# foriequal0/homework-18-graphics-raytracer

Hardware: AMD Instinct MI355X
Metric: Mrays/s (primary+secondary) at 1920x1080, depth 8 (higher is better)
Workload: dtype f32

## Files before the change

### homework-18-graphics-raytracer_amd/csrc/rt_pwf.hip

```cpp
#include "rt_pwf_kernel.h"

namespace rt {

static size_t pwf_dynamic_lds(uint32_t node_cap, uint32_t ring_cap) {
    const bool packed = pa_ready_packed(node_cap, ring_cap);
    return (size_t)(PA_READY_WORDS((node_cap + 63u) / 64u, packed) + 2u * PA_READY_WORDS(ring_cap / 64u, packed)) * sizeof(uint32_t);
}

int pwf_workgroups_per_cu(uint32_t node_cap, uint32_t ring_cap, bool bfs_walk) {
    int n = 0;
    const size_t lds = pwf_dynamic_lds(node_cap, ring_cap);
    const bool packed = pa_ready_packed(node_cap, ring_cap);
    const hipError_t e = bfs_walk ? (packed ? hipOccupancyMaxActiveBlocksPerMultiprocessor(&n, pwf_kernel<true, true>, (int)PA_THREADS, lds)
                                            : hipOccupancyMaxActiveBlocksPerMultiprocessor(&n, pwf_kernel<false, true>, (int)PA_THREADS, lds))
                                  : (packed ? hipOccupancyMaxActiveBlocksPerMultiprocessor(&n, pwf_kernel<true, false>, (int)PA_THREADS, lds)
                                            : hipOccupancyMaxActiveBlocksPerMultiprocessor(&n, pwf_kernel<false, false>, (int)PA_THREADS, lds));
    if (e != hipSuccess || n < 1) n = 1;
    return n;
}

__global__ void pwf_init_kernel(uint32_t *global, KernelFrame *frame, const KernelFrame fr) {
    if (threadIdx.x < PW_G_BLOCK_WORDS) global[threadIdx.x] = 0u;
    if (threadIdx.x == 0u) *frame = fr;
}

size_t pwf_arena_bytes(uint32_t node_cap, uint32_t ring_cap, uint32_t max_depth) {
    return ((size_t)node_cap * 4u + (size_t)ring_cap * (3u + PA_SHADE_U4)) * sizeof(uint4) + (size_t)(node_cap / 64u) * 2u * sizeof(uint32_t) +
           (((size_t)node_cap + 15u) & ~(size_t)15u) + (size_t)pwf_fold_list_regions(max_depth) * node_cap * sizeof(uint32_t) + 256u;
}

#ifdef PA_STATS
static uint32_t *g_pw_last_global = nullptr;
extern "C" int rt_diag_read_pwf(uint32_t *out32) {
    if (!g_pw_last_global) return -1;
    return hipMemcpy(out32, g_pw_last_global, 32 * sizeof(uint32_t), hipMemcpyDeviceToHost) == hipSuccess ? 0 : -1;
}
extern "C" int rt_diag_read_pwf_phases(unsigned long long *out32, int reset) {
    if (hipMemcpyFromSymbol(out32, HIP_SYMBOL(pa_phase_stats), 32 * sizeof(unsigned long long)) != hipSuccess) return -1;
    if (reset) {
        unsigned long long zero[32] = {0};
        if (hipMemcpyToSymbol(HIP_SYMBOL(pa_phase_stats), zero, sizeof zero) != hipSuccess) return -1;
    }
    return 0;
}
#endif

hipError_t launch_pwf(const KernelScene &sc, KernelFrame fr, float *out, const PwParams &pp, uint32_t workgroups, hipStream_t stream,
                      bool init, bool first_band, bool last_band) {
    const uint32_t total = fr.cols * fr.rows;
    fr.n_chunks = (total + 63u) / 64u;
    if (total == 0u) return hipSuccess;
#ifdef PA_STATS
    g_pw_last_global = pp.global;
#endif
    if (init) hipLaunchKernelGGL(pwf_init_kernel, dim3(1), dim3(64), 0, stream, pp.global, const_cast<KernelFrame *>(pp.frame), fr);
    if (first_band) record_main_kernel_event(0, stream);
    const size_t lds = pwf_dynamic_lds(pp.node_cap, pp.ring_cap);
    const bool packed = pa_ready_packed(pp.node_cap, pp.ring_cap);
    if (frame_is_rays(fr)) launch_pwf_rays(sc, pp, out, workgroups, lds, stream, packed, sc.bfs_walk != 0u && pp.bfs_scratch != nullptr);
    else launch_pwf_kernel<false>(sc, pp, out, workgroups, lds, stream, packed, sc.bfs_walk != 0u && pp.bfs_scratch != nullptr);
    if (last_band) record_main_kernel_event(1, stream);
    return hipGetLastError();
}

}

#ifdef RT_DIAG_STAGES
RT_DIAG_STAGE_READER(rt_diag_read_stages_pwf)
#endif
#ifdef RT_DIAG_NEED
RT_DIAG_NEED_READER(rt_diag_read_need_pwf)
#endif
#ifdef RT_DIAG_BFS
RT_DIAG_BFS_READER(rt_diag_read_bfs)
#endif
```

### homework-18-graphics-raytracer_amd/csrc/rt_pwf_common.h

```cpp
#ifndef RT_PWF_COMMON_H
#define RT_PWF_COMMON_H

#include <hip/hip_runtime.h>
#include <stdint.h>

#include "rt_shade.h"
#include "rt_kernels.h"
#include "rt_cast.h"

namespace rt {

#define PW_NO_CHILD 0xffffffffu
#define PW_FINAL 0xfffffffeu
#define PW_DEPTH_SHIFT 21u
#define PW_MODE_SHIFT 27u
#define PW_EXCL_MASK (0xe0000000u | ((1u << PW_DEPTH_SHIFT) - 1u))


__device__ __forceinline__ uint32_t pfu(float x) { return __float_as_uint(x); }
__device__ __forceinline__ float puf(uint32_t x) { return __uint_as_float(x); }

__device__ __forceinline__ uint32_t lds_append(uint32_t *counter, bool want) {
    const unsigned long long mask = __builtin_amdgcn_ballot_w64(want);
    if (mask == 0ull) return 0u;
// ... 67 lines not shown
        const uint32_t c = w & 0xffffu;
        if (c == 64u || (w & PA_SEALED) != 0u) {
            if (atomicCAS(&q->taken, page, page + 1u) == page) {
                ready[page & page_mask] = 0u;
                *start = page * 64u;
                return c;
            }
            continue;
        }
        if (min_partial == 0u || a >= (page + 1u) * 64u || c < min_partial || c != a - page * 64u) return 0u;
        if (atomicCAS(&q->alloc, a, (page + 1u) * 64u) == a) atomicOr(&ready[page & page_mask], PA_SEALED);
    }
    return 0u;
}

PA_HELPER uint32_t pa_try_append(PaQueue *q, const uint32_t *released, uint32_t capacity, bool want, bool *ok) {
    const unsigned long long mask = __builtin_amdgcn_ballot_w64(want);
    *ok = true;
    if (mask == 0ull) return 0u;
    const uint32_t n = (uint32_t)__builtin_popcountll(mask);
    const int leader = (int)__builtin_ctzll(mask);
    uint32_t base = 0xffffffffu;
    if ((int)(threadIdx.x & 63u) == leader) {
        for (int tries = 0; tries < 4; ++tries) {
            const uint32_t a = lds_load(&q->alloc);
            if (a + n - (lds_load(released) << 6) > capacity) break;
            if (atomicCAS(&q->alloc, a, a + n) == a) { base = a; break; }
        }
    }
    base = (uint32_t)__builtin_amdgcn_readlane((int)base, leader);
    if (base == 0xffffffffu) { *ok = false; return 0u; }
    return base + __builtin_amdgcn_mbcnt_hi((uint32_t)(mask >> 32), __builtin_amdgcn_mbcnt_lo((uint32_t)mask, 0u));
}

PA_HELPER uint32_t pa_try_append_some(PaQueue *q, const uint32_t *released, uint32_t capacity, bool want, bool *ok) {
    const unsigned long long mask = __builtin_amdgcn_ballot_w64(want);
    *ok = false;
    if (mask == 0ull) return 0u;
    const uint32_t n = (uint32_t)__builtin_popcountll(mask);
    const int leader = (int)__builtin_ctzll(mask);
    uint32_t base = 0u, take = 0u;
    if ((int)(threadIdx.x & 63u) == leader) {
        for (int tries = 0; tries < 4; ++tries) {
            const uint32_t a = lds_load(&q->alloc);
            const uint32_t used = a - (lds_load(released) << 6);
            const uint32_t t = used >= capacity ? 0u : (capacity - used < n ? capacity - used : n);
            if (t == 0u) break;
            if (atomicCAS(&q->alloc, a, a + t) == a) { base = a; take = t; break; }
        }
    }
    base = (uint32_t)__builtin_amdgcn_readlane((int)base, leader);
    take = (uint32_t)__builtin_amdgcn_readlane((int)take, leader);
    const uint32_t rank = __builtin_amdgcn_mbcnt_hi((uint32_t)(mask >> 32), __builtin_amdgcn_mbcnt_lo((uint32_t)mask, 0u));
    *ok = want && rank < take;
    return base + rank;
}

template <bool PACKED = false>
PA_HELPER void pa_publish(uint32_t *ready, uint32_t page_mask, bool want, uint32_t pos, uint32_t *gen) {
    const unsigned long long mask = __builtin_amdgcn_ballot_w64(want);
    if (mask == 0ull) return;
    __builtin_amdgcn_fence(__ATOMIC_RELEASE, "workgroup");
    const uint32_t n = (uint32_t)__builtin_popcountll(mask);
    const int leader = (int)__builtin_ctzll(mask);
    const uint32_t first = (uint32_t)__builtin_amdgcn_readlane((int)pos, leader);
    if ((int)(threadIdx.x & 63u) == leader) {
        const uint32_t p0 = first >> 6, p1 = (first + n - 1u) >> 6;
        if (PACKED) {
            const uint32_t i0 = p0 & page_mask, i1 = p1 & page_mask;
            const uint32_t n0 = p0 == p1 ? n : (p1 << 6) - first;
            atomicAdd(&ready[i0 >> 1], n0 << pa_ready_shift(i0));
            if (p0 != p1) atomicAdd(&ready[i1 >> 1], (n - n0) << pa_ready_shift(i1));
        } else if (p0 == p1) {
            atomicAdd(&ready[p0 & page_mask], n);
        } else {
            const uint32_t n0 = (p1 << 6) - first;
            atomicAdd(&ready[p0 & page_mask], n0);
            atomicAdd(&ready[p1 & page_mask], n - n0);
        }
        atomicAdd(gen, 1u);
    }
}

template <class Scene>
__device__ __forceinline__ bool next_shadow_ray(const Scene &sc, uint32_t *light_i, V3 pos, V3 adj_n, DirLight *dl) {
    while (*light_i < sc.n_lights) {
        V3 direction;
        if (light_asks(sc.lights[*light_i], sc.light_aux[*light_i], pos, adj_n, &direction)) {
            (void)approximate_into_directional(sc.lights[*light_i], pos, dl);
            return true;
        }
        *light_i += 1u;
    }
    return false;
}

template <class Scene>
__device__ __forceinline__ bool next_shadow_ray_in_step(const Scene &sc, uint32_t first, bool searching, uint32_t *light_i, V3 pos, V3 adj_n) {
    bool found = false;
    for (uint32_t li = first; li < sc.n_lights; ++li) {
        if (__builtin_amdgcn_ballot_w64(searching) == 0ull) break;
        V3 direction;
        const bool asks = light_asks(uniform_ref(sc.lights + li), uniform_ref(sc.light_aux + li), pos, adj_n, &direction);
        if (searching && asks) {
            *light_i = li;
            found = true;
            searching = false;
        }
    }
    return found;
}

}

#endif
```

### homework-18-graphics-raytracer_amd/csrc/rt_pwf_kernel.h

```cpp
#ifndef RT_PWF_KERNEL_H
#define RT_PWF_KERNEL_H

#include <hip/hip_runtime.h>
#include <stdint.h>

#include "../../include/rt_amd.h"
#include "rt_device_scene.h"
#include "rt_shade.h"
#include "rt_kernels.h"
#include "rt_cast.h"
#include "rt_pwf_common.h"

namespace rt {

#ifndef PA_WAVES
#define PA_WAVES 8u
#endif
#define PA_THREADS (PA_WAVES * 64u)
#ifndef PA_MIN_WAVES
#define PA_MIN_WAVES 6
#endif
#ifndef PA_SHADE_PAGES
#define PA_SHADE_PAGES 4u
#endif
#ifndef PA_MIN_PARTIAL
#define PA_MIN_PARTIAL 1u
#endif
#ifndef PA_CHAIN_PARTIAL_MIN
#define PA_CHAIN_PARTIAL_MIN 1u
#endif
#ifndef PA_PRIO_CHAIN
#define PA_PRIO_CHAIN 1
#define PA_PRIO_TILE 1
#endif
#ifndef PA_SLEEP
#define PA_SLEEP 16
#endif
#define PA_SHADE_U4 5u
#ifndef PA_LDS_PAGES
#define PA_LDS_PAGES 2u
#endif
#ifndef PA_LQ
#define PA_LQ 3u
#endif
#define PA_LQ_SHIFT 4u
#ifndef PA_LDS_F_PAGES
#define PA_LDS_F_PAGES 2u
#endif
#ifndef PA_LDS_N_PAGES
#define PA_LDS_N_PAGES 2u
#endif
#ifndef PA_DRAIN_ROOM
#define PA_DRAIN_ROOM 64u
#endif
#define PA_IN_LDS 8u
#define PA_SPIN_LIMIT (1u << 22)

enum : uint32_t { PA_T_NONE = 0u, PA_T_NODE = 1u, PA_T_REFR = 2u, PA_T_TILE = 3u, PA_T_SHADE = 4u };

struct PaShared {
    PaQueue n, f, s;
    PaQueue l[PA_LQ];
    uint32_t l_released[PA_LQ];
    uint32_t ready_l[PA_LQ][PA_LDS_PAGES];
    PaQueue lf;
    uint32_t lf_released;
    uint32_t ready_lf[PA_LDS_F_PAGES];
    PaQueue ln;
    uint32_t ln_released;
    uint32_t ready_ln[PA_LDS_N_PAGES];
    uint32_t root_alloc;
    uint32_t tiles_exhausted;
    uint32_t tile_list_count;
    uint32_t static_next;
    uint32_t idle;
    uint32_t gen;
    uint32_t done;
    uint32_t abort;
    uint32_t fold_count[64];
};

template <class P>
__device__ __forceinline__ void pa_store_shade(P *t, uint32_t id, uint32_t prim, uint32_t word, V3 spos, V3 adj_n, V3 in_dir, V3 sdiffuse, V3 sum) {
    t[PA_F(0u)] = make_uint4(id, prim, word, 0u);
    t[PA_F(1u)] = make_uint4(pfu(spos.x), pfu(spos.y), pfu(spos.z), pfu(sum.x));
    t[PA_F(2u)] = make_uint4(pfu(adj_n.x), pfu(adj_n.y), pfu(adj_n.z), pfu(sum.y));
    t[PA_F(3u)] = make_uint4(pfu(in_dir.x), pfu(in_dir.y), pfu(in_dir.z), pfu(sum.z));
    t[PA_F(4u)] = make_uint4(pfu(sdiffuse.x), pfu(sdiffuse.y), pfu(sdiffuse.z), 0u);
}

template <class P>
__device__ __forceinline__ void pa_store_node(P *t, V3 o, V3 d, uint32_t word, float contribution, uint32_t id) {
    t[PA_F(0u)] = make_uint4(pfu(o.x), pfu(o.y), pfu(o.z), pfu(d.x));
    t[PA_F(1u)] = make_uint4(pfu(d.y), pfu(d.z), word, pfu(contribution));
    if (id != 0xffffffffu) t[PA_F(2u)] = make_uint4(id, 0u, 0u, 0u);
}

__device__ __forceinline__ uint32_t pa_top_node(uint32_t *root_alloc, const uint32_t *n_alloc, uint32_t node_cap, bool want, bool *overflow) {
    const unsigned long long mask = __builtin_amdgcn_ballot_w64(want);
    *overflow = false;
    if (mask == 0ull) return 0u;
    const uint32_t n = (uint32_t)__builtin_popcountll(mask);
    const int leader = (int)__builtin_ctzll(mask);
    uint32_t base = 0u;
    if ((int)(threadIdx.x & 63u) == leader) base = atomicAdd(root_alloc, n);
    base = (uint32_t)__builtin_amdgcn_readlane((int)base, leader);
    if (base + n + lds_load(n_alloc) > node_cap) { *overflow = want; return 0u; }
    return node_cap - 1u - (base + __builtin_amdgcn_mbcnt_hi((uint32_t)(mask >> 32), __builtin_amdgcn_mbcnt_lo((uint32_t)mask, 0u)));
}

template <class P>
__device__ __forceinline__ void pa_store_refr(P *t, V3 o, V3 d, uint32_t word, uint32_t parent, uint32_t obj, float contribution, float travel, uint32_t retry) {
    t[PA_F(0u)] = make_uint4(pfu(o.x), pfu(o.y), pfu(o.z), pfu(d.x));
    t[PA_F(1u)] = make_uint4(pfu(d.y), pfu(d.z), word, parent);
    t[PA_F(2u)] = make_uint4(obj, pfu(contribution), pfu(travel), retry);
}

__device__ __forceinline__ void pa_release_page(uint32_t *released, uint32_t page, uint32_t lane) {
    asm volatile("s_waitcnt lgkmcnt(0)" ::: "memory");
    if (lane == 0u) {
        while (lds_load(released) != page) __builtin_amdgcn_s_sleep(1);
        __hip_atomic_store(released, page + 1u, __ATOMIC_RELEASE, __HIP_MEMORY_SCOPE_WORKGROUP);
    }
}

#ifdef PA_STATS
__device__ unsigned long long pa_phase_stats[32];
#define PA_TICK() __builtin_readcyclecounter()
#endif

template <bool PACKED, bool BFS = false, bool RAYS = false>
__global__ __launch_bounds__(PA_THREADS, BFS ? 2 : PA_MIN_WAVES) void pwf_kernel(const KernelScene sc, const PwParams pp, float *__restrict__ out) {
    BfsLds *bfs_lds = nullptr;
    BfsScratch bfs_ws = {nullptr, nullptr, nullptr, 0u, 0u};
    if constexpr (BFS) {
        __shared__ BfsLds bfs_lds_all[PA_WAVES];
        bfs_lds = &bfs_lds_all[threadIdx.x >> 6];
        uint2 *const mine = reinterpret_cast<uint2 *>(pp.bfs_scratch) + ((size_t)blockIdx.x * PA_WAVES + (threadIdx.x >> 6)) * (2u * (size_t)pp.bfs_items_cap + pp.bfs_jobs_cap);
        bfs_ws.items_a = mine;
        bfs_ws.items_b = mine + pp.bfs_items_cap;
        bfs_ws.jobs = mine + 2u * (size_t)pp.bfs_items_cap;
        bfs_ws.items_cap = pp.bfs_items_cap;
        bfs_ws.jobs_cap = pp.bfs_jobs_cap;
    }
    extern __shared__ uint32_t pa_ready[];
    __shared__ PaShared S;
    __shared__ uint4 lds_shade[PA_LQ * PA_LDS_PAGES * PA_SHADE_U4 * 64u];
    __shared__ uint4 lds_refr[PA_LDS_F_PAGES * 3u * 64u];
    __shared__ uint4 lds_node[PA_LDS_N_PAGES * 3u * 64u];
    const auto &fr = uniform_ref(pp.frame);
    const uint32_t lane = threadIdx.x & 63u;
    const uint32_t total_slots = fr.cols * fr.rows;
    const uint32_t n_tiles = fr.n_chunks;
    const float THRESHOLD = 0.001f;

    unsigned char *arena = pp.arena + (size_t)blockIdx.x * pp.arena_stride;
    uint4 *node_in = reinterpret_cast<uint4 *>(arena);
    uint4 *nodes = node_in + (size_t)pp.node_cap * 2u;
    uint4 *shade_q = nodes + (size_t)pp.node_cap * 2u;
    uint4 *refr_q = shade_q + (size_t)pp.ring_cap * PA_SHADE_U4;
    uint32_t *tile_list = reinterpret_cast<uint32_t *>(refr_q + (size_t)pp.ring_cap * 3u);
    const uint32_t ring_mask = pp.ring_cap - 1u;
    const uint32_t tile_cap = pp.node_cap / 64u;
    unsigned char *root_mark = reinterpret_cast<unsigned char *>(((uintptr_t)(tile_list + (size_t)tile_cap * 2u) + 15u) & ~(uintptr_t)15u);
    uint32_t *fold_list = reinterpret_cast<uint32_t *>(root_mark + (((size_t)pp.node_cap + 15u) & ~(size_t)15u));
    auto fold_slot = [&](uint32_t level, uint32_t i) -> uint32_t * {
        uint32_t *region = fold_list + (size_t)((level - 1u) >> 1) * pp.node_cap;
        return region + (((level - 1u) & 1u) != 0u ? pp.node_cap - 1u - i : i);
    };
    const uint32_t node_pages = (pp.node_cap + 63u) / 64u, ring_pages = pp.ring_cap / 64u;
    uint32_t *ready_n = pa_ready, *ready_s = pa_ready + PA_READY_WORDS(node_pages, PACKED), *ready_f = ready_s + PA_READY_WORDS(ring_pages, PACKED);
    const uint32_t ring_page_mask = ring_pages - 1u;

    for (uint32_t i = threadIdx.x; i < PA_READY_WORDS(node_pages, PACKED) + 2u * PA_READY_WORDS(ring_pages, PACKED); i += PA_THREADS) pa_ready[i] = 0u;
    if (threadIdx.x < 64u) S.fold_count[threadIdx.x] = 0u;
    if (threadIdx.x == 0u) {
        S.n.alloc = S.n.taken = 0u;
        S.f.alloc = S.f.taken = 0u;
        S.s.alloc = S.s.taken = 0u;
        for (uint32_t q = 0; q < PA_LQ; ++q) {
            S.l[q].alloc = S.l[q].taken = 0u;
            S.l_released[q] = 0u;
            for (uint32_t k = 0; k < PA_LDS_PAGES; ++k) S.ready_l[q][k] = 0u;
        }
        S.lf.alloc = S.lf.taken = 0u;
        S.lf_released = 0u;
        for (uint32_t k = 0; k < PA_LDS_F_PAGES; ++k) S.ready_lf[k] = 0u;
        S.ln.alloc = S.ln.taken = 0u;
        S.ln_released = 0u;
        for (uint32_t k = 0; k < PA_LDS_N_PAGES; ++k) S.ready_ln[k] = 0u;
        S.root_alloc = 0u;
        S.tiles_exhausted = 0u;
        S.tile_list_count = 0u;
        S.static_next = 0u;
        S.idle = 0u;
        S.gen = 0u;
        S.done = 0u;
        S.abort = 0u;
    }
    __syncthreads();
    uint32_t casts = 0u;
    auto queue_shade = [&](bool want, uint32_t id, uint32_t prim, uint32_t word, uint32_t light_i, V3 spos, V3 adj_n, V3 in_dir, V3 sdiffuse, V3 sum) {
        const uint32_t mine = light_i < PA_LQ - 1u ? light_i : PA_LQ - 1u;
#pragma unroll
        for (uint32_t q = 0; q < PA_LQ; ++q) {
            const bool w = want && mine == q;
            if (__builtin_amdgcn_ballot_w64(w) == 0ull) continue;
            bool fits;
            const uint32_t k = pa_try_append_some(&S.l[q], &S.l_released[q], PA_LDS_PAGES * 64u, w, &fits);
            if (fits) pa_store_shade(lds_shade + q * (PA_LDS_PAGES * PA_SHADE_U4 * 64u) + pa_entry(k & (PA_LDS_PAGES * 64u - 1u), PA_SHADE_U4), id, prim, word, spos, adj_n, in_dir, sdiffuse, sum);
            pa_publish(S.ready_l[q], PA_LDS_PAGES - 1u, fits, k, &S.gen);
            want = want && !fits;
        }
#ifdef PA_STATS
        for (uint32_t q = 0; q < 3u; ++q) {
            const unsigned long long m = __builtin_amdgcn_ballot_w64(want && (mine < 2u ? mine : 2u) == q);
            if (m != 0ull && lane == (uint32_t)__builtin_ctzll(m)) atomicAdd(pp.global + 28 + q, (uint32_t)__builtin_popcountll(m));
        }
#endif
        const uint32_t k = lds_append(&S.s.alloc, want);
        if (want) pa_store_shade(shade_q + pa_entry(k & ring_mask, PA_SHADE_U4), id, prim, word, spos, adj_n, in_dir, sdiffuse, sum);
        pa_publish<PACKED>(ready_s, ring_page_mask, want, k, &S.gen);
    };
#ifdef PA_STATS
    const unsigned long long st_t0 = __builtin_amdgcn_s_memrealtime();
    uint32_t st_hist[5] = {0u, 0u, 0u, 0u, 0u};
    uint32_t st_shadow[3] = {0u, 0u, 0u};
    unsigned long long ph[26];
    for (int k = 0; k < 26; ++k) ph[k] = 0ull;
#endif

    for (;;) {
        if (lds_load(&S.done) != 0u || lds_load(&S.abort) != 0u) break;

#ifdef PA_STATS
        const unsigned long long ph_t0 = PA_TICK();
#endif
        uint32_t type = PA_T_NONE, start = 0u, count = 0u;
        if (lane == 0u) {
            const uint32_t gen = lds_load(&S.gen);
            auto look = [&]() -> uint32_t {
                const uint32_t a0 = lds_load(&S.ln.alloc), a1 = lds_load(&S.n.alloc), a2 = lds_load(&S.lf.alloc), a3 = lds_load(&S.f.alloc);
                const uint32_t t0 = lds_load(&S.ln.taken), t1 = lds_load(&S.n.taken), t2 = lds_load(&S.lf.taken), t3 = lds_load(&S.f.taken);
                uint32_t al[PA_LQ], tl[PA_LQ];
                for (uint32_t q = 0; q < PA_LQ; ++q) { al[q] = lds_load(&S.l[q].alloc); tl[q] = lds_load(&S.l[q].taken); }
                const uint32_t as = lds_load(&S.s.alloc), ts = lds_load(&S.s.taken);
                uint32_t m = (a0 > t0 * 64u ? 1u : 0u) | (a1 > t1 * 64u ? 2u : 0u) | (a2 > t2 * 64u ? 4u : 0u) | (a3 > t3 * 64u ? 8u : 0u);
                for (uint32_t q = 0; q < PA_LQ; ++q) m |= al[q] > tl[q] * 64u ? 16u << q : 0u;
                m |= as > ts * 64u ? 16u << PA_LQ : 0u;
                return m;
            };
            uint32_t have = look();
            auto claim_chain = [&](uint32_t min_partial) {
                if ((have & 1u) != 0u) {
                    count = pa_claim(&S.ln, S.ready_ln, PA_LDS_N_PAGES - 1u, min_partial, &start);
                    if (count != 0u) { type = PA_T_NODE | PA_IN_LDS; return; }
                }
                if ((have & 2u) != 0u) {
                    count = pa_claim<PACKED>(&S.n, ready_n, 0xffffffffu, min_partial, &start);
                    if (count != 0u) { type = PA_T_NODE; return; }
                }
                if ((have & 4u) != 0u) {
                    count = pa_claim(&S.lf, S.ready_lf, PA_LDS_F_PAGES - 1u, min_partial, &start);
                    if (count != 0u) { type = PA_T_REFR | PA_IN_LDS; return; }
                }
                if ((have & 8u) != 0u) {
                    count = pa_claim<PACKED>(&S.f, ready_f, ring_page_mask, min_partial, &start);
                    if (count != 0u) type = PA_T_REFR;
                }
            };
            auto claim_shade = [&](uint32_t min_partial) {
                for (uint32_t q = 0; q < PA_LQ; ++q) {
                    if ((have & (16u << q)) == 0u) continue;
                    count = pa_claim(&S.l[q], S.ready_l[q], PA_LDS_PAGES - 1u, min_partial, &start);
                    if (count != 0u) { type = PA_T_SHADE | PA_IN_LDS | (q << PA_LQ_SHIFT); return; }
                }
                if ((have & (16u << PA_LQ)) == 0u) return;
                count = pa_claim<PACKED>(&S.s, ready_s, ring_page_mask, min_partial, &start);
                if (count != 0u) type = PA_T_SHADE;
            };
            claim_chain(0u);
            if (PA_DRAIN_ROOM != 0u && type == PA_T_NONE && lds_load(&S.tiles_exhausted) == 0u) {
                for (uint32_t q = 0; q < PA_LQ; ++q) {
                    if (lds_load(&S.l[q].alloc) - (lds_load(&S.l_released[q]) << 6) + PA_DRAIN_ROOM > PA_LDS_PAGES * 64u) {
                        count = pa_claim(&S.l[q], S.ready_l[q], PA_LDS_PAGES - 1u, 0u, &start);
                        if (count != 0u) { type = PA_T_SHADE | PA_IN_LDS | (q << PA_LQ_SHIFT); break; }
                    }
                }
            }
            if (PA_CHAIN_PARTIAL_MIN != 0u && type == PA_T_NONE) claim_chain(PA_CHAIN_PARTIAL_MIN);
            bool tried_tile = false;
            for (int pass = 0; pass < 2 && type == PA_T_NONE; ++pass) {
                if (!tried_tile && lds_load(&S.tiles_exhausted) == 0u) {
                    uint32_t shade_pages = (lds_load(&S.s.alloc) >> 6) - lds_load(&S.s.taken);
                    for (uint32_t q = 0; q < PA_LQ; ++q) shade_pages += (lds_load(&S.l[q].alloc) >> 6) - lds_load(&S.l[q].taken);
                    if (pass == 1 || (int32_t)shade_pages < (int32_t)PA_SHADE_PAGES) {
                        tried_tile = true;
                        const uint32_t used = lds_load(&S.n.alloc) + lds_load(&S.root_alloc);
                        const uint32_t room = pp.node_cap > used ? pp.node_cap - used : 0u;
                        if (room < 64u * pp.tile_reserve || lds_load(&S.tile_list_count) >= tile_cap) {
                            S.tiles_exhausted = 1u;
                        } else {
                            const uint32_t share = n_tiles / gridDim.x;
                            const uint32_t own = share / 2u > (share < 8u ? share : 8u) ? share / 2u : (share < 8u ? share : 8u);
                            uint32_t k;
                            const uint32_t mine = own != 0u && lds_load(&S.static_next) < own ? atomicAdd(&S.static_next, 1u) : own;
                            if (mine < own) k = blockIdx.x + gridDim.x * mine;
                            else k = gridDim.x * own + atomicAdd(pp.global + PW_G_TILE, 1u);
                            if (k >= n_tiles) {
                                S.tiles_exhausted = 1u;
                            } else {
                                start = pp.tile_order != nullptr ? pp.tile_order[k] : (uint32_t)(((unsigned long long)k * pp.tile_stride) % n_tiles);
                                count = total_slots - start * 64u < 64u ? total_slots - start * 64u : 64u;
                                type = PA_T_TILE;
                            }
                        }
                    }
                }
                if (type == PA_T_NONE && pass == 0) claim_shade(0u);
            }
            for (int last = 0; last < 2 && type == PA_T_NONE; ++last) {
                const uint32_t min_partial = last ? 1u : PA_MIN_PARTIAL;
                have = look();
                claim_chain(min_partial);
                if (type != PA_T_NONE) break;
                claim_shade(min_partial);
                if (type != PA_T_NONE) break;
                if (last) {
                    if (lds_load(&S.idle) == PA_WAVES - 1u) S.done = 1u;
                    break;
                }
                if (atomicAdd(&S.idle, 1u) + 1u == PA_WAVES) {
                    atomicSub(&S.idle, 1u);
                    continue;
                }
                uint32_t spins = 0u;
                while (lds_load(&S.gen) == gen && lds_load(&S.done) == 0u && lds_load(&S.abort) == 0u) {
                    __builtin_amdgcn_s_sleep(PA_SLEEP);
                    if (++spins > PA_SPIN_LIMIT) {
                        S.abort = 1u;
                        atomicExch(pp.global + PW_G_OVERFLOW, 1u);
                    }
                }
                atomicSub(&S.idle, 1u);
                break;
            }
        }
        type = (uint32_t)__builtin_amdgcn_readfirstlane((int)type);
        start = (uint32_t)__builtin_amdgcn_readfirstlane((int)start);
        count = (uint32_t)__builtin_amdgcn_readfirstlane((int)count);
        const bool in_lds = (type & PA_IN_LDS) != 0u;
        const uint32_t lq = (type >> PA_LQ_SHIFT) & 3u;
        type &= 7u;
        const bool one_light = type == PA_T_SHADE && in_lds && (lq < PA_LQ - 1u || sc.n_lights <= PA_LQ);
#ifdef PA_STATS
        const unsigned long long ph_t1 = PA_TICK();
        if (type == PA_T_NONE) ph[24] += ph_t1 - ph_t0;
        const uint32_t ph_k = type == PA_T_NODE ? 0u : (type == PA_T_REFR ? 1u : (type == PA_T_TILE ? 2u : 3u));
#endif
        if (type == PA_T_NONE) continue;
        __builtin_amdgcn_fence(__ATOMIC_ACQUIRE, "workgroup");
        if (type == PA_T_SHADE) __builtin_amdgcn_s_setprio(0);
        else if (type == PA_T_TILE) __builtin_amdgcn_s_setprio(PA_PRIO_TILE);
        else __builtin_amdgcn_s_setprio(PA_PRIO_CHAIN);
#ifdef PA_STATS
        st_hist[count <= 8u ? 0 : (count <= 16u ? 1 : (count <= 32u ? 2 : (count < 64u ? 3 : 4)))] += 1u;
#endif

        const bool active = lane < count;
        Ray req;
        req.o = v3(0.0f, 0.0f, 0.0f);
        req.d = v3(0.0f, 0.0f, 1.0f);
        req.mode = FACE_FRONT;
        req.excl = 0u;
        bool do_cast = active;
        uint32_t id = 0u;
        uint32_t depth = 0u;
        float contribution = 1.0f;
        uint32_t obj = 0u;
        float travel = 0.0f;
        int32_t retry = -1;
        uint32_t prim = 0u, light_i = 0u, sflags = 0u;
        V3 spos = v3(0.0f, 0.0f, 0.0f), adj_n = v3(0.0f, 0.0f, 1.0f), in_dir = v3(0.0f, 0.0f, 1.0f), sdiffuse = spos, sum = spos;
        DirLight dl;
        dl.direction = dl.color = v3(0.0f, 0.0f, 0.0f);
        bool from_tile = false;

        if (type == PA_T_TILE) {
            const uint32_t tile = start;
            uint32_t base = 0u, entry = 0u;
            if (lane == 0u) {
                base = atomicAdd(&S.root_alloc, count);
                entry = atomicAdd(&S.tile_list_count, 1u);
            }
            base = (uint32_t)__builtin_amdgcn_readfirstlane((int)base);
            entry = (uint32_t)__builtin_amdgcn_readfirstlane((int)entry);
            if (base + count + lds_load(&S.n.alloc) > pp.node_cap || entry >= tile_cap) {
                if (lane == 0u) { S.abort = 1u; atomicExch(pp.global + PW_G_OVERFLOW, 1u); }
                break;
            }
            const uint32_t first_id = pp.node_cap - base - count;
            if (lane == 0u) { tile_list[entry * 2u] = tile; tile_list[entry * 2u + 1u] = first_id; }
            id = first_id + lane;
            depth = (uint32_t)(fr.max_depth > 0 ? fr.max_depth : 0);
            if constexpr (RAYS) {
                contribution = frame_root_contribution(fr);
                if (active) req = ray_from_abi(frame_rays(fr) + (tile * 64u + lane), sc.n_triangles, sc.n_spheres);
                do_cast = active && !(contribution < THRESHOLD);
            } else if (active) {
                uint32_t row, col;
                pw_slot_to_pixel(fr, tile * 64u + lane, &row, &col);
                const uint32_t x = fr.x0 + col, y = fr.y0 + row * fr.y_step;
                const float clip_y = (fr.half_height - (float)y) / fr.height_f;
                const float clip_x = ((float)x - fr.half_width) / fr.height_f;
                const V3 cx = v3(fr.cam_x[0], fr.cam_x[1], fr.cam_x[2]);
                const V3 cy = v3(fr.cam_y[0], fr.cam_y[1], fr.cam_y[2]);
                const V3 ct = v3(fr.cam_toward[0], fr.cam_toward[1], fr.cam_toward[2]);
                req.o = v3(fr.cam_origin[0], fr.cam_origin[1], fr.cam_origin[2]);
                req.d = normalize(clip_x * cx + clip_y * cy + ct);
            }
            type = PA_T_NODE;
            from_tile = true;
        } else if (type == PA_T_NODE) {
            uint4 a, b;
            a = b = make_uint4(0u, 0u, 0u, 0u);
            if (in_lds) {
                if (active) {
                    const uint4 *t = lds_node + pa_entry((start + lane) & (PA_LDS_N_PAGES * 64u - 1u), 3u);
                    a = t[PA_F(0u)], b = t[PA_F(1u)];
                    id = t[PA_F(2u)].x;
                }
                pa_release_page(&S.ln_released, start >> 6, lane);
            } else {
                id = start + lane;
                if (active) a = node_in[pa_entry(id, 2u)], b = node_in[pa_entry(id, 2u) + PA_F(1u)];
            }
            if (active) {
                req.o = v3(puf(a.x), puf(a.y), puf(a.z));
                req.d = v3(puf(a.w), puf(b.x), puf(b.y));
                req.mode = (b.z >> PW_MODE_SHIFT) & 3u;
                depth = (b.z >> PW_DEPTH_SHIFT) & 63u;
                req.excl = b.z & PW_EXCL_MASK;
                contribution = puf(b.w);
            }
        } else if (type == PA_T_REFR) {
            uint4 a, b, c;
            a = b = c = make_uint4(0u, 0u, 0u, 0u);
            if (in_lds) {
                if (active) {
                    const uint4 *t = lds_refr + pa_entry((start + lane) & (PA_LDS_F_PAGES * 64u - 1u), 3u);
                    a = t[PA_F(0u)], b = t[PA_F(1u)], c = t[PA_F(2u)];
                }
                pa_release_page(&S.lf_released, start >> 6, lane);
            } else if (active) {
                const uint4 *t = refr_q + pa_entry((start + lane) & ring_mask, 3u);
                a = t[PA_F(0u)], b = t[PA_F(1u)], c = t[PA_F(2u)];
            }
            if (active) {
                req.o = v3(puf(a.x), puf(a.y), puf(a.z));
                req.d = v3(puf(a.w), puf(b.x), puf(b.y));
                req.mode = (b.z >> PW_MODE_SHIFT) & 3u;
                depth = (b.z >> PW_DEPTH_SHIFT) & 63u;
                req.excl = b.z & PW_EXCL_MASK;
                id = b.w;
                obj = c.x;
                contribution = puf(c.y);
                travel = puf(c.z);
                retry = (int32_t)c.w;
            }
        } else {
            uint4 a, b, c, d, e;
            a = b = c = d = e = make_uint4(0u, 0u, 0u, 0u);
            if (in_lds) {
                if (active) {
                    const uint4 *t = lds_shade + lq * (PA_LDS_PAGES * PA_SHADE_U4 * 64u) + pa_entry((start + lane) & (PA_LDS_PAGES * 64u - 1u), PA_SHADE_U4);
                    a = t[PA_F(0u)], b = t[PA_F(1u)], c = t[PA_F(2u)], d = t[PA_F(3u)], e = t[PA_F(4u)];
                }
                pa_release_page(&S.l_released[lq], start >> 6, lane);
            } else if (active) {
                const uint4 *t = shade_q + pa_entry((start + lane) & ring_mask, PA_SHADE_U4);
                a = t[PA_F(0u)], b = t[PA_F(1u)], c = t[PA_F(2u)], d = t[PA_F(3u)], e = t[PA_F(4u)];
            }
            if (active) {
                id = a.x; prim = a.y; obj = a.z & 0xffffu; light_i = (a.z >> 16) & 0x3fffu; sflags = a.z >> 30;
                spos = v3(puf(b.x), puf(b.y), puf(b.z)); sum.x = puf(b.w);
                adj_n = v3(puf(c.x), puf(c.y), puf(c.z)); sum.y = puf(c.w);
                in_dir = v3(puf(d.x), puf(d.y), puf(d.z)); sum.z = puf(d.w);
                sdiffuse = v3(puf(e.x), puf(e.y), puf(e.z));
                if (one_light) do_cast = approximate_into_directional(uniform_ref(sc.lights + lq), spos, &dl);
                else do_cast = next_shadow_ray(sc, &light_i, spos, adj_n, &dl);
                req.o = spos;
                req.d = -dl.direction;
                req.mode = FACE_BACK;
                req.excl = pack_excl(prim, FACE_BACK);
            }
        }

#ifdef PA_STATS
        const unsigned long long ph_t2 = PA_TICK();
#endif
        CastResult cr;
        cr.prim = -1;
        cr.t = 0.0f;
        cr.bf = 0u;
        cr.a0 = cr.a1 = cr.a2 = 0.0f;
        if constexpr (BFS) {
            cr = cast_bfs(sc, req, do_cast, bfs_lds, bfs_ws);
            if (do_cast) casts += 1u;
        } else if (do_cast) {
            cr = cast_asm(sc, req);
            casts += 1u;
        }
#ifdef PA_STATS
        const unsigned long long ph_t3 = PA_TICK();
#endif

        if (type == PA_T_NODE) {
            V3 acc = v3(0.0f, 0.0f, 0.0f);
            float rc = 0.0f, fc = 0.0f;
            uint32_t rec_cr = PW_FINAL, rec_cf = PW_NO_CHILD;
            bool want_shade = false, want_refl = false, want_refr = false;
            HitGeom nh;
            nh.pos = nh.normal = v3(0.0f, 0.0f, 0.0f);
            nh.u = nh.v = 0.0f;
            nh.prim = nh.bf = nh.obj = 0u;
            V3 inside_d = v3(0.0f, 0.0f, 0.0f);
            if (active && cr.prim >= 0) {
                nh = finish_hit(sc, req, cr, false);
                const rt_material &rm = sc.materials[nh.obj];
                const float shade_contribution = (1.0f - rm.shiness) * (1.0f - rm.transparency);
                want_shade = contribution * shade_contribution >= THRESHOLD;
                if (depth > 0u) {
                    acc = v3(0.0f, 0.0f, 0.0f) * shade_contribution;
                    rc = rm.shiness * (1.0f - rm.transparency);
                    fc = rm.transparency;
                    rec_cr = PW_NO_CHILD;
                    want_refl = contribution * rc >= THRESHOLD;
                    if (contribution * fc > THRESHOLD) {
                        V3 refract_in;
                        if (refract_dir(nh.normal, req.d, rm.refraction_index, &refract_in)) {
                            inside_d = normalize(refract_in);
                            want_refr = true;
                        }
                    }
                }
            }
            bool refl_in_lds, overflow;
            const uint32_t q_refl = pa_try_append(&S.ln, &S.ln_released, PA_LDS_N_PAGES * 64u, want_refl, &refl_in_lds);
            const uint32_t k_refl = refl_in_lds ? pa_top_node(&S.root_alloc, &S.n.alloc, pp.node_cap, want_refl, &overflow)
                                                : lds_append(&S.n.alloc, want_refl);
            if (!refl_in_lds) overflow = want_refl && k_refl + lds_load(&S.root_alloc) >= pp.node_cap;
            if (want_refl && !overflow) rec_cr = k_refl;
            const bool below = active && cr.prim >= 0 && depth > 0u && (want_refl || want_refr);
            const bool bare = active && cr.prim >= 0 && depth > 0u && !below;
            if (active) {
                if (below) nodes[pa_entry(id, 2u) + PA_F(1u)] = make_uint4(pfu(fc), 0u, rec_cr, rec_cf);
                if (from_tile) root_mark[id] = (unsigned char)(below ? 0u : 0xffu);
            }
            if (want_refl && !overflow) {
                const V3 d = reflect_dir(nh.normal, req.d);
                const uint32_t word = pack_excl(nh.prim, nh.bf ? FACE_FRONT : FACE_BACK) | (req.mode << PW_MODE_SHIFT) | ((depth - 1u) << PW_DEPTH_SHIFT);
                if (refl_in_lds) pa_store_node(lds_node + pa_entry(q_refl & (PA_LDS_N_PAGES * 64u - 1u), 3u), nh.pos, d, word, contribution * rc, k_refl);
                else pa_store_node(node_in + pa_entry(k_refl, 2u), nh.pos, d, word, contribution * rc, 0xffffffffu);
            }
// ... 244 lines not shown
                    const uint32_t nv = total_slots - first_slot < 64u ? total_slots - first_slot : 64u;
                    live[j] = lane < nv;
                    id[j] = base + lane;
                    slot[j] = first_slot + lane;
                }
                if (live[j]) {
                    ra[j] = nodes[pa_entry(id[j], 2u)];
                    rb[j] = make_uint4(0u, 0u, PW_FINAL, PW_NO_CHILD);
                    if (root_mark[id[j]] != 0xffu) rb[j] = nodes[pa_entry(id[j], 2u) + PA_F(1u)];
                }
            }
            if (pp.tile_cost != nullptr) {
#pragma unroll
                for (uint32_t j = 0; j < 4u; ++j) {
                    const unsigned long long deep = __builtin_amdgcn_ballot_w64(live[j] && rb[j].z != PW_FINAL);
                    if (lane == 0u && tile_of[j] != 0xffffffffu) pp.tile_cost[tile_of[j]] = (uint32_t)__builtin_popcountll(deep);
                }
            }
            uint4 cr4[4], cf4[4];
#pragma unroll
            for (uint32_t j = 0; j < 4u; ++j) {
                cr4[j] = cf4[j] = make_uint4(0u, 0u, 0u, 0u);
                if (live[j] && rb[j].z != PW_FINAL) {
                    if (rb[j].z != PW_NO_CHILD) cr4[j] = nodes[pa_entry(rb[j].z, 2u)];
                    if (rb[j].w != PW_NO_CHILD) cf4[j] = nodes[pa_entry(rb[j].w, 2u)];
                }
            }
#pragma unroll
            for (uint32_t j = 0; j < 4u; ++j) {
                if (!live[j]) continue;
                const uint4 a = ra[j], b = rb[j];
                V3 value = v3(puf(a.x), puf(a.y), puf(a.z));
                if (b.z != PW_FINAL) {
                    const float rc = puf(a.w), fc = puf(b.x), decay = puf(b.y);
                    V3 reflection = v3(0.0f, 0.0f, 0.0f), refraction = v3(0.0f, 0.0f, 0.0f);
                    if (b.z != PW_NO_CHILD) reflection = v3(puf(cr4[j].x), puf(cr4[j].y), puf(cr4[j].z));
                    if (b.w != PW_NO_CHILD) refraction = v3(puf(cf4[j].x), puf(cf4[j].y), puf(cf4[j].z)) * decay;
                    value = (value + reflection * rc) + refraction * fc;
                }
                uint32_t row, col;
                pw_slot_to_pixel(fr, slot[j], &row, &col);
                float *px = out + ((size_t)row * fr.cols + col) * 3u;
                if constexpr (RAYS) {
                    px[0] = value.x;
                    px[1] = value.y;
                    px[2] = value.z;
                } else {
                    px[0] = 0.0f + value.x;
                    px[1] = 0.0f + value.y;
                    px[2] = 0.0f + value.z;
                }
            }
        }
        if (threadIdx.x == 0u && n_started != 0u) atomicAdd(pp.global + PW_G_TILES_DONE, n_started);
#ifdef PA_STATS
        __syncthreads();
        if (threadIdx.x == 0u) {
            atomicAdd(&pa_phase_stats[26], st_f0 - st_t2);
            atomicAdd(&pa_phase_stats[27], st_f1 - st_f0);
            atomicAdd(&pa_phase_stats[28], __builtin_amdgcn_s_memrealtime() - st_f1);
            atomicAdd(&pa_phase_stats[29], 1ull);
        }
#endif
    }
#ifdef PA_STATS
    __syncthreads();
    {
        const unsigned long long st_t3 = __builtin_amdgcn_s_memrealtime();
        if (lane == 0u) { atomicAdd(pp.global + 8, (uint32_t)(st_t1 - st_t0)); atomicMax(pp.global + 9, (uint32_t)(st_t1 - st_t0)); }
        if (lane == 0u) for (int k = 0; k < 5; ++k) atomicAdd(pp.global + 20 + k, st_hist[k]);
        for (int k = 0; k < 3; ++k) {
            uint32_t v = st_shadow[k];
            for (int off = 32; off > 0; off >>= 1) v += __shfl_down(v, off, 64);
            if (lane == 0u && v != 0u) atomicAdd(pp.global + (k == 0 ? 18 : (k == 1 ? 19 : 31)), v);
        }
        if (lane == 0u) {
            ph[25] = st_t3 - st_t2;
            for (int k = 0; k < 26; ++k) atomicAdd(&pa_phase_stats[k], ph[k]);
        }
        if (threadIdx.x == 0u) {
            atomicAdd(pp.global + 10, (uint32_t)(st_t2 - st_t0)); atomicMax(pp.global + 11, (uint32_t)(st_t2 - st_t0));
            atomicAdd(pp.global + 12, (uint32_t)(st_t3 - st_t2)); atomicMax(pp.global + 13, (uint32_t)(st_t3 - st_t2));
            atomicAdd(pp.global + 14, 1u); atomicAdd(pp.global + 15, S.n.alloc);
            atomicAdd(pp.global + 25, S.s.alloc); atomicAdd(pp.global + 26, S.f.alloc); atomicAdd(pp.global + 27, S.root_alloc);
            atomicMin(pp.global + 16, (uint32_t)(st_t3 - st_t0)); atomicMax(pp.global + 17, (uint32_t)(st_t3 - st_t0));
        }
    }
#endif
    if (threadIdx.x == 0u) S.gen = 0u;
    __syncthreads();
    for (int off = 32; off > 0; off >>= 1) casts += __shfl_down(casts, off, 64);
    if (lane == 0u && casts != 0u) atomicAdd(&S.gen, casts);

    __syncthreads();
    if (threadIdx.x == 0u) {
        if (S.gen != 0u) atomicAdd(reinterpret_cast<unsigned long long *>(pp.global + PW_G_CASTS), (unsigned long long)S.gen);
        __threadfence();
        if (atomicAdd(pp.global + PW_G_GROUPS_DONE, 1u) + 1u == gridDim.x) {
            __threadfence();
            uint32_t overflow = __hip_atomic_load(pp.global + PW_G_OVERFLOW, __ATOMIC_RELAXED, __HIP_MEMORY_SCOPE_AGENT);
            const uint32_t tiles_done = __hip_atomic_load(pp.global + PW_G_TILES_DONE, __ATOMIC_RELAXED, __HIP_MEMORY_SCOPE_AGENT);
            if (overflow == 0u && tiles_done != n_tiles) {
                overflow = 1u;
                atomicExch(pp.global + PW_G_OVERFLOW, 1u);
            }
            if (overflow == 0u && pp.ray_count != nullptr)
                atomicAdd(pp.ray_count,
                          __hip_atomic_load(reinterpret_cast<unsigned long long *>(pp.global + PW_G_CASTS), __ATOMIC_RELAXED, __HIP_MEMORY_SCOPE_AGENT));
            for (uint32_t k = 0; k < PW_G_BLOCK_WORDS; ++k) pp.global_next[k] = 0u;
        }
    }
}

template <bool RAYS>
static void launch_pwf_kernel(const KernelScene &sc, const PwParams &pp, float *out, uint32_t workgroups, size_t lds, hipStream_t stream, bool packed,
                              bool bfs) {
    if (bfs) {
        if (packed) hipLaunchKernelGGL((pwf_kernel<true, true, RAYS>), dim3(workgroups), dim3(PA_THREADS), lds, stream, sc, pp, out);
        else hipLaunchKernelGGL((pwf_kernel<false, true, RAYS>), dim3(workgroups), dim3(PA_THREADS), lds, stream, sc, pp, out);
    } else if (packed) hipLaunchKernelGGL((pwf_kernel<true, false, RAYS>), dim3(workgroups), dim3(PA_THREADS), lds, stream, sc, pp, out);
    else hipLaunchKernelGGL((pwf_kernel<false, false, RAYS>), dim3(workgroups), dim3(PA_THREADS), lds, stream, sc, pp, out);
}

}

#endif
```

Baseline: 18900.

## Replace linear SHADE ring with per-light-class paged ring and full-page FIFO

Replaces the single linear shade queue in global memory with a paged ring. Each light class owns its own open page, full pages go to an LDS FIFO, and a page is freed once its entries have been read. Because every shade page now holds one light class, the one-light directional fast path also applies to global shade pages, not only LDS ones. This adds LDS FIFO words, CAS loops for page allocation, an overflow abort path, and a full vmcnt wait before each page is freed.

New measurement: 19040 (median of 6 runs). About the same (+0.8%).

```diff
diff --git a/homework-18-graphics-raytracer_amd/csrc/rt_pwf.hip b/homework-18-graphics-raytracer_amd/csrc/rt_pwf.hip
--- a/homework-18-graphics-raytracer_amd/csrc/rt_pwf.hip
+++ b/homework-18-graphics-raytracer_amd/csrc/rt_pwf.hip
@@ -4,7 +4,8 @@
 
 static size_t pwf_dynamic_lds(uint32_t node_cap, uint32_t ring_cap) {
     const bool packed = pa_ready_packed(node_cap, ring_cap);
-    return (size_t)(PA_READY_WORDS((node_cap + 63u) / 64u, packed) + 2u * PA_READY_WORDS(ring_cap / 64u, packed)) * sizeof(uint32_t);
+    return (size_t)(PA_READY_WORDS((node_cap + 63u) / 64u, packed) + 2u * PA_READY_WORDS(ring_cap / 64u, packed) + PA_RING_FIFO_WORDS(ring_cap / 64u, packed)) *
+           sizeof(uint32_t);
 }
 
 int pwf_workgroups_per_cu(uint32_t node_cap, uint32_t ring_cap, bool bfs_walk) {
@@ -35,10 +36,10 @@
     if (!g_pw_last_global) return -1;
     return hipMemcpy(out32, g_pw_last_global, 32 * sizeof(uint32_t), hipMemcpyDeviceToHost) == hipSuccess ? 0 : -1;
 }
-extern "C" int rt_diag_read_pwf_phases(unsigned long long *out32, int reset) {
-    if (hipMemcpyFromSymbol(out32, HIP_SYMBOL(pa_phase_stats), 32 * sizeof(unsigned long long)) != hipSuccess) return -1;
+extern "C" int rt_diag_read_pwf_phases(unsigned long long *out40, int reset) {
+    if (hipMemcpyFromSymbol(out40, HIP_SYMBOL(pa_phase_stats), PA_PHASE_WORDS * sizeof(unsigned long long)) != hipSuccess) return -1;
     if (reset) {
-        unsigned long long zero[32] = {0};
+        unsigned long long zero[PA_PHASE_WORDS] = {0};
         if (hipMemcpyToSymbol(HIP_SYMBOL(pa_phase_stats), zero, sizeof zero) != hipSuccess) return -1;
     }
     return 0;
diff --git a/homework-18-graphics-raytracer_amd/csrc/rt_pwf_common.h b/homework-18-graphics-raytracer_amd/csrc/rt_pwf_common.h
--- a/homework-18-graphics-raytracer_amd/csrc/rt_pwf_common.h
+++ b/homework-18-graphics-raytracer_amd/csrc/rt_pwf_common.h
@@ -173,6 +173,131 @@
     }
 }
 
+#define PA_RING_INUSE 0x4000u
+#define PA_RING_COUNT 0x7fu
+#define PA_RING_ENTRY 0x8000u
+#define PA_RING_NONE 0xffffffffu
+#define PA_RING_FIFO_WORDS(pages, packed) ((packed) ? ((pages) + 1u) / 2u : 0u)
+
+template <bool PACKED>
+struct PaRing {
+    PaQueue *q;
+    uint32_t *page_alloc;
+    uint32_t *cur;
+    uint32_t *ready, *fifo;
+    uint32_t page_mask;
+
+    PA_HELPER uint32_t *state_word(uint32_t slot) const { return PACKED ? &ready[slot >> 1] : &ready[slot]; }
+    PA_HELPER uint32_t state_shift(uint32_t slot) const { return PACKED ? pa_ready_shift(slot) : 0u; }
+    PA_HELPER uint32_t *fifo_word(uint32_t i) const { return PACKED ? &fifo[i >> 1] : &ready[i]; }
+    PA_HELPER uint32_t fifo_shift(uint32_t i) const { return PACKED ? pa_ready_shift(i) : 16u; }
+    PA_HELPER uint32_t state(uint32_t slot) const { return (lds_load(state_word(slot)) >> state_shift(slot)) & 0xffffu; }
+
+    PA_HELPER uint32_t page() const {
+        for (uint32_t tries = 0; tries <= page_mask; ++tries) {
+            const uint32_t seq = atomicAdd(page_alloc, 1u);
+            uint32_t *w = state_word(seq & page_mask);
+            const uint32_t sh = state_shift(seq & page_mask);
+            for (;;) {
+                const uint32_t o = lds_load(w);
+                if (((o >> sh) & 0xffffu) != 0u) break;
+                if (atomicCAS(w, o, o | (PA_RING_INUSE << sh)) == o) return seq;
+            }
+        }
+        return PA_RING_NONE;
+    }
+    PA_HELPER void free_page(uint32_t slot) const { atomicAnd(state_word(slot), ~(0xffffu << state_shift(slot))); }
+
+    PA_HELPER uint32_t reserve(uint32_t cls, bool want, uint32_t *p0, uint32_t *n0, uint32_t *p1, uint32_t *n1, bool *ok) const {
+        const unsigned long long mask = __builtin_amdgcn_ballot_w64(want);
+        *ok = true;
+        *p0 = *p1 = *n0 = *n1 = 0u;
+        if (mask == 0ull) return 0u;
+        const uint32_t n = (uint32_t)__builtin_popcountll(mask);
+        const int leader = (int)__builtin_ctzll(mask);
+        uint32_t a = PA_RING_NONE, spare = PA_RING_NONE, room = 0u;
+        if ((int)(threadIdx.x & 63u) == leader) {
+            bool done = false;
+            for (int tries = 0; tries < 64 && !done; ++tries) {
+                a = lds_load(&cur[cls]);
+                room = a == PA_RING_NONE ? 0u : 64u - (a & 63u);
+                uint32_t next;
+                if (n < room) next = a + n;
+                else if (n == room) next = PA_RING_NONE;
+                else {
+                    if (spare == PA_RING_NONE) spare = page();
+                    if (spare == PA_RING_NONE) break;
+                    next = n - room == 64u ? PA_RING_NONE : (spare << 6) + (n - room);
+                }
+                done = atomicCAS(&cur[cls], a, next) == a;
+            }
+            if (spare != PA_RING_NONE && (!done || n <= room)) {
+                free_page(spare & page_mask);
+                spare = PA_RING_NONE;
+            }
+            if (!done) room = 0xffffffffu;
+        }
+        a = (uint32_t)__builtin_amdgcn_readlane((int)a, leader);
+        spare = (uint32_t)__builtin_amdgcn_readlane((int)spare, leader);
+        room = (uint32_t)__builtin_amdgcn_readlane((int)room, leader);
+        if (room == 0xffffffffu) { *ok = false; return 0u; }
+        const uint32_t rank = __builtin_amdgcn_mbcnt_hi((uint32_t)(mask >> 32), __builtin_amdgcn_mbcnt_lo((uint32_t)mask, 0u));
+        *n0 = n < room ? n : room;
+        *n1 = n - *n0;
+        *p0 = a >> 6;
+        *p1 = spare;
+        return rank < room ? a + rank : (spare << 6) + (rank - room);
+    }
+
+    PA_HELPER void count_in(uint32_t seq, uint32_t n, uint32_t cls) const {
+        const uint32_t slot = seq & page_mask;
+        const uint32_t old = (atomicAdd(state_word(slot), n << state_shift(slot)) >> state_shift(slot)) & PA_RING_COUNT;
+        if (old + n != 64u) return;
+        const uint32_t i = atomicAdd(&q->alloc, 1u) & page_mask;
+        atomicOr(fifo_word(i), (PA_RING_ENTRY | (cls << 12) | slot) << fifo_shift(i));
+    }
+    PA_HELPER void publish(uint32_t cls, bool want, uint32_t p0, uint32_t n0, uint32_t p1, uint32_t n1, uint32_t *gen) const {
+        const unsigned long long mask = __builtin_amdgcn_ballot_w64(want);
+        if (mask == 0ull) return;
+        __builtin_amdgcn_fence(__ATOMIC_RELEASE, "workgroup");
+        if ((int)(threadIdx.x & 63u) == (int)__builtin_ctzll(mask)) {
+            if (n0 != 0u) count_in(p0, n0, cls);
+            if (n1 != 0u) count_in(p1, n1, cls);
+            atomicAdd(gen, 1u);
+        }
+    }
+
+    PA_HELPER uint32_t claim_full(uint32_t *start, uint32_t *cls) const {
+        for (int tries = 0; tries < 4; ++tries) {
+            const uint32_t t = lds_load(&q->taken);
+            if ((int32_t)(lds_load(&q->alloc) - t) <= 0) return 0u;
+            const uint32_t i = t & page_mask;
+            const uint32_t e = (lds_load(fifo_word(i)) >> fifo_shift(i)) & 0xffffu;
+            if (e == 0u) return 0u;
+            if (atomicCAS(&q->taken, t, t + 1u) == t) {
+                atomicAnd(fifo_word(i), ~(0xffffu << fifo_shift(i)));
+                *start = (e & 0xfffu) << 6;
+                *cls = (e >> 12) & 3u;
+                return 64u;
+            }
+        }
+        return 0u;
+    }
+    PA_HELPER uint32_t claim_open(uint32_t classes, uint32_t min_partial, uint32_t *start, uint32_t *cls) const {
+        for (uint32_t c = 0; c < classes; ++c) {
+            const uint32_t a = lds_load(&cur[c]);
+            if (a == PA_RING_NONE) continue;
+            const uint32_t fill = a & 63u, slot = (a >> 6) & page_mask;
+            if (fill < min_partial || (state(slot) & PA_RING_COUNT) != fill) continue;
+            if (atomicCAS(&cur[c], a, PA_RING_NONE) != a) continue;
+            *start = slot << 6;
+            *cls = c;
+            return fill;
+        }
+        return 0u;
+    }
+};
+
 template <class Scene>
 __device__ __forceinline__ bool next_shadow_ray(const Scene &sc, uint32_t *light_i, V3 pos, V3 adj_n, DirLight *dl) {
     while (*light_i < sc.n_lights) {
diff --git a/homework-18-graphics-raytracer_amd/csrc/rt_pwf_kernel.h b/homework-18-graphics-raytracer_amd/csrc/rt_pwf_kernel.h
--- a/homework-18-graphics-raytracer_amd/csrc/rt_pwf_kernel.h
+++ b/homework-18-graphics-raytracer_amd/csrc/rt_pwf_kernel.h
@@ -60,6 +60,8 @@
 
 struct PaShared {
     PaQueue n, f, s;
+    uint32_t s_page_alloc;
+    uint32_t s_cur[PA_LQ];
     PaQueue l[PA_LQ];
     uint32_t l_released[PA_LQ];
     uint32_t ready_l[PA_LQ][PA_LDS_PAGES];
@@ -125,7 +127,8 @@
 }
 
 #ifdef PA_STATS
-__device__ unsigned long long pa_phase_stats[32];
+#define PA_PHASE_WORDS 40
+__device__ unsigned long long pa_phase_stats[PA_PHASE_WORDS];
 #define PA_TICK() __builtin_readcyclecounter()
 #endif
 
@@ -171,14 +174,19 @@
     const uint32_t node_pages = (pp.node_cap + 63u) / 64u, ring_pages = pp.ring_cap / 64u;
     uint32_t *ready_n = pa_ready, *ready_s = pa_ready + PA_READY_WORDS(node_pages, PACKED), *ready_f = ready_s + PA_READY_WORDS(ring_pages, PACKED);
     const uint32_t ring_page_mask = ring_pages - 1u;
-
-    for (uint32_t i = threadIdx.x; i < PA_READY_WORDS(node_pages, PACKED) + 2u * PA_READY_WORDS(ring_pages, PACKED); i += PA_THREADS) pa_ready[i] = 0u;
+    static_assert(PA_WAVES + PA_LQ <= 1024u / 64u && PA_LQ <= 4u, "the SHADE ring's slack (pw_plan: ring_cap = node_cap + 1024)");
+    const PaRing<PACKED> ring = {&S.s, &S.s_page_alloc, S.s_cur, ready_s, ready_f + PA_READY_WORDS(ring_pages, PACKED), ring_page_mask};
+
+    for (uint32_t i = threadIdx.x; i < PA_READY_WORDS(node_pages, PACKED) + 2u * PA_READY_WORDS(ring_pages, PACKED) + PA_RING_FIFO_WORDS(ring_pages, PACKED); i += PA_THREADS)
+        pa_ready[i] = 0u;
     if (threadIdx.x < 64u) S.fold_count[threadIdx.x] = 0u;
     if (threadIdx.x == 0u) {
         S.n.alloc = S.n.taken = 0u;
         S.f.alloc = S.f.taken = 0u;
         S.s.alloc = S.s.taken = 0u;
+        S.s_page_alloc = 0u;
         for (uint32_t q = 0; q < PA_LQ; ++q) {
+            S.s_cur[q] = PA_RING_NONE;
             S.l[q].alloc = S.l[q].taken = 0u;
             S.l_released[q] = 0u;
             for (uint32_t k = 0; k < PA_LDS_PAGES; ++k) S.ready_l[q][k] = 0u;
@@ -215,12 +223,24 @@
 #ifdef PA_STATS
         for (uint32_t q = 0; q < 3u; ++q) {
             const unsigned long long m = __builtin_amdgcn_ballot_w64(want && (mine < 2u ? mine : 2u) == q);
-            if (m != 0ull && lane == (uint32_t)__builtin_ctzll(m)) atomicAdd(pp.global + 28 + q, (uint32_t)__builtin_popcountll(m));
-        }
-#endif
-        const uint32_t k = lds_append(&S.s.alloc, want);
-        if (want) pa_store_shade(shade_q + pa_entry(k & ring_mask, PA_SHADE_U4), id, prim, word, spos, adj_n, in_dir, sdiffuse, sum);
-        pa_publish<PACKED>(ready_s, ring_page_mask, want, k, &S.gen);
+            if (m != 0ull && lane == (uint32_t)__builtin_ctzll(m)) { atomicAdd(pp.global + 28 + q, (uint32_t)__builtin_popcountll(m)); atomicAdd(pp.global + 25, (uint32_t)__builtin_popcountll(m)); }
+        }
+#endif
+        if (__builtin_amdgcn_ballot_w64(want) == 0ull) return;
+#pragma nounroll
+        for (uint32_t q = 0; q < PA_LQ; ++q) {
+            const bool w = want && mine == q;
+            if (__builtin_amdgcn_ballot_w64(w) == 0ull) continue;
+            uint32_t p0, n0, p1, n1;
+            bool ok;
+            const uint32_t k = ring.reserve(q, w, &p0, &n0, &p1, &n1, &ok);
+            if (!ok) {
+                if (lane == 0u) { S.abort = 1u; atomicExch(pp.global + PW_G_OVERFLOW, 1u); }
+                return;
+            }
+            if (w) pa_store_shade(shade_q + pa_entry(k & ring_mask, PA_SHADE_U4), id, prim, word, spos, adj_n, in_dir, sdiffuse, sum);
+            ring.publish(q, w, p0, n0, p1, n1, &S.gen);
+        }
     };
 #ifdef PA_STATS
     const unsigned long long st_t0 = __builtin_amdgcn_s_memrealtime();
@@ -245,9 +265,11 @@
                 uint32_t al[PA_LQ], tl[PA_LQ];
                 for (uint32_t q = 0; q < PA_LQ; ++q) { al[q] = lds_load(&S.l[q].alloc); tl[q] = lds_load(&S.l[q].taken); }
                 const uint32_t as = lds_load(&S.s.alloc), ts = lds_load(&S.s.taken);
+                uint32_t open = 0u;
+                for (uint32_t q = 0; q < PA_LQ; ++q) open |= ~lds_load(&S.s_cur[q]);
                 uint32_t m = (a0 > t0 * 64u ? 1u : 0u) | (a1 > t1 * 64u ? 2u : 0u) | (a2 > t2 * 64u ? 4u : 0u) | (a3 > t3 * 64u ? 8u : 0u);
                 for (uint32_t q = 0; q < PA_LQ; ++q) m |= al[q] > tl[q] * 64u ? 16u << q : 0u;
-                m |= as > ts * 64u ? 16u << PA_LQ : 0u;
+                m |= as != ts || open != 0u ? 16u << PA_LQ : 0u;
                 return m;
             };
             uint32_t have = look();
@@ -276,8 +298,10 @@
                     if (count != 0u) { type = PA_T_SHADE | PA_IN_LDS | (q << PA_LQ_SHIFT); return; }
                 }
                 if ((have & (16u << PA_LQ)) == 0u) return;
-                count = pa_claim<PACKED>(&S.s, ready_s, ring_page_mask, min_partial, &start);
-                if (count != 0u) type = PA_T_SHADE;
+                uint32_t cls = 0u;
+                count = ring.claim_full(&start, &cls);
+                if (count == 0u && min_partial != 0u) count = ring.claim_open(PA_LQ, min_partial, &start, &cls);
+                if (count != 0u) type = PA_T_SHADE | (cls << PA_LQ_SHIFT);
             };
             claim_chain(0u);
             if (PA_DRAIN_ROOM != 0u && type == PA_T_NONE && lds_load(&S.tiles_exhausted) == 0u) {
@@ -292,7 +316,7 @@
             bool tried_tile = false;
             for (int pass = 0; pass < 2 && type == PA_T_NONE; ++pass) {
                 if (!tried_tile && lds_load(&S.tiles_exhausted) == 0u) {
-                    uint32_t shade_pages = (lds_load(&S.s.alloc) >> 6) - lds_load(&S.s.taken);
+                    uint32_t shade_pages = lds_load(&S.s.alloc) - lds_load(&S.s.taken);
                     for (uint32_t q = 0; q < PA_LQ; ++q) shade_pages += (lds_load(&S.l[q].alloc) >> 6) - lds_load(&S.l[q].taken);
                     if (pass == 1 || (int32_t)shade_pages < (int32_t)PA_SHADE_PAGES) {
                         tried_tile = true;
@@ -352,7 +376,7 @@
         const bool in_lds = (type & PA_IN_LDS) != 0u;
         const uint32_t lq = (type >> PA_LQ_SHIFT) & 3u;
         type &= 7u;
-        const bool one_light = type == PA_T_SHADE && in_lds && (lq < PA_LQ - 1u || sc.n_lights <= PA_LQ);
+        const bool one_light = type == PA_T_SHADE && (lq < PA_LQ - 1u || sc.n_lights <= PA_LQ);
 #ifdef PA_STATS
         const unsigned long long ph_t1 = PA_TICK();
         if (type == PA_T_NONE) ph[24] += ph_t1 - ph_t0;
@@ -477,9 +501,16 @@
                     a = t[PA_F(0u)], b = t[PA_F(1u)], c = t[PA_F(2u)], d = t[PA_F(3u)], e = t[PA_F(4u)];
                 }
                 pa_release_page(&S.l_released[lq], start >> 6, lane);
-            } else if (active) {
-                const uint4 *t = shade_q + pa_entry((start + lane) & ring_mask, PA_SHADE_U4);
-                a = t[PA_F(0u)], b = t[PA_F(1u)], c = t[PA_F(2u)], d = t[PA_F(3u)], e = t[PA_F(4u)];
+            } else {
+                if (active) {
+                    const uint4 *t = shade_q + pa_entry((start + lane) & ring_mask, PA_SHADE_U4);
+                    a = t[PA_F(0u)], b = t[PA_F(1u)], c = t[PA_F(2u)], d = t[PA_F(3u)], e = t[PA_F(4u)];
+                }
+                asm volatile("s_waitcnt vmcnt(0)" ::: "memory");
+                if (lane == 0u) ring.free_page(start >> 6);
+#ifdef PA_STATS
+                if (lane == 0u) { atomicAdd(&pa_phase_stats[32u + (lq < 2u ? lq : 2u)], 1ull); if (!one_light) atomicAdd(&pa_phase_stats[35], 1ull); }
+#endif
             }
             if (active) {
                 id = a.x; prim = a.y; obj = a.z & 0xffffu; light_i = (a.z >> 16) & 0x3fffu; sflags = a.z >> 30;
@@ -890,7 +921,7 @@
             atomicAdd(pp.global + 10, (uint32_t)(st_t2 - st_t0)); atomicMax(pp.global + 11, (uint32_t)(st_t2 - st_t0));
             atomicAdd(pp.global + 12, (uint32_t)(st_t3 - st_t2)); atomicMax(pp.global + 13, (uint32_t)(st_t3 - st_t2));
             atomicAdd(pp.global + 14, 1u); atomicAdd(pp.global + 15, S.n.alloc);
-            atomicAdd(pp.global + 25, S.s.alloc); atomicAdd(pp.global + 26, S.f.alloc); atomicAdd(pp.global + 27, S.root_alloc);
+            atomicAdd(pp.global + 26, S.f.alloc); atomicAdd(pp.global + 27, S.root_alloc);
             atomicMin(pp.global + 16, (uint32_t)(st_t3 - st_t0)); atomicMax(pp.global + 17, (uint32_t)(st_t3 - st_t0));
         }
     }
```
